# nighting0le01/On_Device_Image_Captioning

Measured on AMD Instinct MI355X. Metric: captions/sec end-to-end (Swin-L 384, beam=3) at 1/2/4/8 MI355X, higher is better.
Workload: dtype bf16; 1 GPU; End_ExpansionNet_v2 end-to-end, Swin-L/384 backbone, batch 16 per GPU, beam 3, beam_max_seq_len 20 (BASELINE.json configs[2]); workload_key=e2e16, batch_per_gpu=16, beam=3, beam_max_seq_len=20, decoder_steps=19, weights=synthetic xavier (Philox, seed 0), backbone_precision=bf16, encoder_precision=bf16, decoder_precision=fp32, hip_graphs=True, parallelism=image-shard x1, caption_len_check=20, encode_lanes=1, decode_lanes=2, decode_cus=0, decode_group_batches=1

## Files before the change

### include/odic_hip.h

```cpp
#ifndef ODIC_HIP_H
#define ODIC_HIP_H

#include <stddef.h>
#include <stdint.h>

#ifdef __cplusplus
extern "C" {
#endif

#define ODIC_F32 0
#define ODIC_BF16 1
#define ODIC_FP8 2
#define ODIC_F16 3
#define ODIC_H2 4

#define ODIC_ACT_NONE 0
#define ODIC_ACT_GELU 1
#define ODIC_ACT_RELU 2
#define ODIC_ACT_SIGMOID 3

#define ODIC_EINVAL (-1)
#define ODIC_ENULL (-2)
#define ODIC_EUNSUPPORTED (-3)

#define ODIC_ABI_VERSION 23
int odic_abi_version(void);

const char* odic_build_info(void);

typedef struct odic_gemm_args {
  const void* A; const void* W; const float* bias; const float* residual; void* out;
  int32_t M, N, K;
  int64_t lda, ldw, ldr, ldc;
  int32_t batch;
  int64_t strideA, strideW, strideBias, strideR, strideC;
  float alpha;
  int32_t act;
  int32_t bias_axis;
  int32_t in_dtype;
  int32_t out_dtype;
  int32_t tile_cfg;
  const float* ln_colsum; float ln_eps;
  int32_t* workspace;
  const float* col_scale; float out_scale;
  void* out16; int64_t ld16; float* stats_out;
  const float* ln_stats;
  const float* a_ln; int64_t ld_aln;
} odic_gemm_args;
int odic_gemm(const odic_gemm_args* args, void* stream);

int odic_layernorm(const float* x, int64_t ldx, const float* gamma, const float* beta, void* out,
                   int32_t M, int32_t C, float eps, int32_t out_dtype, void* stream);

int odic_copy(const void* src, void* dst, int64_t nbytes, void* stream);

int odic_cast_f32_to_bf16(const float* x, int64_t ldx, void* out, int64_t ldo, int32_t M, int32_t C,
                          void* stream);
int odic_cast_f32_to_h2(const float* x, int64_t ldx, void* out, int64_t ldo, int32_t M, int32_t C, void* stream);
// ... 76 lines not shown
} odic_jpeg_scan;

typedef struct odic_jpeg_prog_batch {
  const void* headers;
  const void* scans;
  const void* tables;
  const uint8_t* data;
  uint8_t* out;
  int32_t* status;
  int32_t n_images, n_scans, n_tables, n_levels, max_width, max_height, pad0, pad1;
  int64_t max_blocks, total_scan_bytes, total_intervals, total_blocks, total_plane_bytes;
  int32_t level_first[ODIC_JPEG_MAX_SCANS + 1];
  int32_t level_intervals[ODIC_JPEG_MAX_SCANS];
  int32_t pad2;
} odic_jpeg_prog_batch;

size_t odic_jpeg_progressive_workspace_bytes(const odic_jpeg_prog_batch* batch);

size_t odic_jpeg_progressive_coef_offset(const odic_jpeg_prog_batch* batch);

int odic_jpeg_decode_progressive(const odic_jpeg_prog_batch* batch, void* workspace, size_t ws_bytes, void* stream);

int odic_jpeg_decode_progressive_scaled(const odic_jpeg_prog_batch* batch, const int32_t* scale_log2, void* workspace,
                                        size_t ws_bytes, void* stream);

int odic_window_attention(const void* qkv, const float* bias_table, const float* bias_shifted_prescaled,
                          void* out, int32_t B, int32_t res, int32_t C, int32_t heads, int32_t ws,
                          int32_t shift, float scale, int32_t dtype, void* stream);

int odic_swin_qkv_attention(const float* x, int64_t ldx, const void* w_qkv_folded, const float* b_qkv_folded,
                            const float* bias_shifted_prescaled, void* out, int32_t B, int32_t res, int32_t C,
                            int32_t heads, int32_t ws, int32_t shift, float scale, float ln_eps, void* stream);

int odic_swin_mlp(const float* x, int64_t ldx, const void* w1_folded, const float* b1_folded, const void* w2,
                  const float* b2, float alpha2, float* out, int64_t ldo, int32_t M, int32_t C, float ln_eps,
                  void* stream);

int odic_stcexp_normalize(const float* z, const int32_t* enc_len, const int32_t* group_meta,
                          int32_t ngroups, void* pos_fw, void* neg_fw, int64_t ld_fw, void* pos_bw,
                          void* neg_bw, int64_t ld_bw, float* colsum_ws, int32_t B, int32_t nq,
                          int32_t S, float eps, float scale_fw, float scale_bw, int32_t out_dtype, void* stream);

int odic_selector_mix(const float* x, int64_t ldx, const float* sel_pre, int64_t lds,
                      const float* a, int64_t lda, const float* b, int64_t ldb, float* out,
                      int64_t ldo, int32_t M, int32_t d, void* stream);


int odic_dec_embed(const int64_t* tokens, const float* embed, const float* pos_table,
                   const int32_t* pos, float* y, int64_t ldy, int32_t N, int32_t d, int32_t pos_rows,
                   float scale, void* stream);

int odic_dynexp_step(const float* lin, int64_t ldlin, const float* qexp, const float* bexp,
                     float* cond_c, float* key_c, float* va_c, float* vb_c, float* wfa_c,
                     float* wfb_c, float* qk_c, const int32_t* anc, const int32_t* row_valid,
                     const int32_t* pos, const float* y_in, int64_t ldy_in, float* y, int64_t ldy,
                     int32_t N, int32_t T, int32_t d, int32_t E, float eps, void* stream);


int odic_dec_embed_seq(const int64_t* tokens, const float* embed, const float* pos_table, const int32_t* dec_len,
                       int32_t* row_valid, float* y, int64_t ldy, int32_t N, int32_t T, int32_t d, int32_t vocab,
                       int32_t pos_rows, float scale, void* stream);

int odic_dynexp_seq(const float* lin, int64_t ldlin, const float* qexp, const float* bexp, const int32_t* dec_len,
                    const float* y_in, int64_t ldy_in, float* y, int64_t ldy, int32_t N, int32_t T, int32_t d,
                    int32_t E, float eps, void* stream);

// ... 54 lines not shown
```

### on_device_image_captioning_amd/_hip.py

```python
from __future__ import annotations

import ctypes as C
import os

_HERE = os.path.dirname(os.path.abspath(__file__))
LIB_PATH = os.path.join(_HERE, "libodic_hip.so")

F32, BF16, FP8, F16, H2 = 0, 1, 2, 3, 4
ACT_NONE, ACT_GELU, ACT_RELU, ACT_SIGMOID = 0, 1, 2, 3
ABI_VERSION = 23

_ERR = {-1: "ODIC_EINVAL (bad shape / alignment / enum)", -2: "ODIC_ENULL (required pointer is NULL)",
        -3: "ODIC_EUNSUPPORTED"}


class GemmArgs(C.Structure):
    _fields_ = [("A", C.c_void_p), ("W", C.c_void_p), ("bias", C.c_void_p), ("residual", C.c_void_p),
                ("out", C.c_void_p),
                ("M", C.c_int32), ("N", C.c_int32), ("K", C.c_int32),
                ("lda", C.c_int64), ("ldw", C.c_int64), ("ldr", C.c_int64), ("ldc", C.c_int64),
                ("batch", C.c_int32),
                ("strideA", C.c_int64), ("strideW", C.c_int64), ("strideBias", C.c_int64),
                ("strideR", C.c_int64), ("strideC", C.c_int64),
                ("alpha", C.c_float), ("act", C.c_int32), ("bias_axis", C.c_int32),
                ("in_dtype", C.c_int32), ("out_dtype", C.c_int32), ("tile_cfg", C.c_int32),
                ("ln_colsum", C.c_void_p), ("ln_eps", C.c_float), ("workspace", C.c_void_p),
                ("col_scale", C.c_void_p), ("out_scale", C.c_float),
                ("out16", C.c_void_p), ("ld16", C.c_int64), ("stats_out", C.c_void_p), ("ln_stats", C.c_void_p),
                ("a_ln", C.c_void_p), ("ld_aln", C.c_int64)]


class BeamState(C.Structure):
    _fields_ = [(n, C.c_void_p) for n in
                ("tokens", "logprobs", "anc", "cumul", "n_elem", "has_eos", "row_valid", "next_tok",
                 "pos", "done", "ctr")]


class EmbedArgs(C.Structure):
    _fields_ = [("embed", C.c_void_p), ("pos_table", C.c_void_p), ("y", C.c_void_p), ("ldy", C.c_int64),
                ("d", C.c_int32), ("scale", C.c_float), ("pos_rows", C.c_int32)]


class JpegBatch(C.Structure):
# ... 7 lines not shown


JPEG_MAX_SCANS = 64


class JpegProgBatch(C.Structure):
    _fields_ = [("headers", C.c_void_p), ("scans", C.c_void_p), ("tables", C.c_void_p), ("data", C.c_void_p),
                ("out", C.c_void_p), ("status", C.c_void_p),
                ("n_images", C.c_int32), ("n_scans", C.c_int32), ("n_tables", C.c_int32), ("n_levels", C.c_int32),
                ("max_width", C.c_int32), ("max_height", C.c_int32), ("pad0", C.c_int32), ("pad1", C.c_int32),
                ("max_blocks", C.c_int64), ("total_scan_bytes", C.c_int64), ("total_intervals", C.c_int64),
                ("total_blocks", C.c_int64), ("total_plane_bytes", C.c_int64),
                ("level_first", C.c_int32 * (JPEG_MAX_SCANS + 1)), ("level_intervals", C.c_int32 * JPEG_MAX_SCANS),
                ("pad2", C.c_int32)]


_P, _I32, _I64, _F = C.c_void_p, C.c_int32, C.c_int64, C.c_float

_SIGNATURES = {
    "odic_abi_version": (C.c_int, []),
    "odic_build_info": (C.c_char_p, []),
    "odic_gemm": (C.c_int, [C.POINTER(GemmArgs), _P]),
    "odic_layernorm": (C.c_int, [_P, _I64, _P, _P, _P, _I32, _I32, _F, _I32, _P]),
    "odic_cast_f32_to_bf16": (C.c_int, [_P, _I64, _P, _I64, _I32, _I32, _P]),
    "odic_cast_f32_to_h2": (C.c_int, [_P, _I64, _P, _I64, _I32, _I32, _P]),
    "odic_patch_merge_layernorm": (C.c_int, [_P, _P, _P, _P, _I32, _I32, _I32, _F, _I32, _P]),
    "odic_patch_embed": (C.c_int, [_P] * 6 + [_I32] * 6 + [_F, _P]),
    "odic_resize_bilinear_normalize": (C.c_int, [_P, _I32, _I32, _I64, _P, _P, _I32, _P, _P, _I32, _P, _P, _I32,
                                                 C.POINTER(C.c_float), C.POINTER(C.c_float), _P]),
    "odic_resize_boxes_normalize": (C.c_int, [_P, _I32, _P, _P, _P, _P, C.c_size_t, _P, _I32, _I32,
                                              C.POINTER(C.c_float), C.POINTER(C.c_float), _P]),
    "odic_window_attention": (C.c_int, [_P, _P, _P, _P] + [_I32] * 6 + [_F, _I32, _P]),
    "odic_swin_qkv_attention": (C.c_int, [_P, _I64, _P, _P, _P, _P] + [_I32] * 6 + [_F, _F, _P]),
    "odic_swin_mlp": (C.c_int, [_P, _I64, _P, _P, _P, _P, _F, _P, _I64, _I32, _I32, _F, _P]),
    "odic_stcexp_normalize": (C.c_int, [_P, _P, _P, _I32, _P, _P, _I64, _P, _P, _I64, _P, _I32, _I32, _I32, _F, _F, _F, _I32,
                                        _P]),
    "odic_selector_mix": (C.c_int, [_P, _I64, _P, _I64, _P, _I64, _P, _I64, _P, _I64, _I32, _I32, _P]),
    "odic_copy": (C.c_int, [_P, _P, _I64, _P]),
    "odic_dec_embed": (C.c_int, [_P, _P, _P, _P, _P, _I64, _I32, _I32, _I32, _F, _P]),
    "odic_dec_embed_seq": (C.c_int, [_P, _P, _P, _P, _P, _P, _I64] + [_I32] * 5 + [_F, _P]),
    "odic_dynexp_seq": (C.c_int, [_P, _I64, _P, _P, _P, _P, _I64, _P, _I64] + [_I32] * 4 + [_F, _P]),
    "odic_token_stats": (C.c_int, [_P, _I64, _P, _P, _P, _P, _P, _P, _I32, _I32, _P]),
    "odic_dynexp_step": (C.c_int, [_P, _I64, _P, _P] + [_P] * 7 + [_P, _P, _P, _P, _I64, _P, _I64] + [_I32] * 4 + [_F, _P]),
    "odic_cross_attn_step": (C.c_int, [_P, _I64, _P, _I64, _I32, _I32, _P, _P, _P, _I64] + [_I32] * 5 + [_P]),
    "odic_cross_attn_probs": (C.c_int, [_P, _I64, _P, _I64, _I32, _P, _P, _P, _I64] + [_I32] * 7 + [_F, _P]),
    "odic_logsoftmax_topk": (C.c_int, [_P, _I64, _P, _I64, _P, _P, _I32, _I32, _I32, _P]),
    "odic_logsoftmax_sample": (C.c_int, [_P, _I64, _P, _I64, _P, _P, _I32, _I32, _I32, C.c_uint64, _P, _P]),
    "odic_ensemble_logprobs": (C.c_int, [C.POINTER(C.c_void_p), _I32, _I64, _P, _I64, _I32, _I32, _P]),
    "odic_topk_rows": (C.c_int, [_P, _I64, _P, _P, _I32, _I32, _I32, _P]),
    "odic_beam_step": (C.c_int, [_P, _P, C.POINTER(BeamState), C.POINTER(EmbedArgs), _I32, _I32, _I32, _I64, _P]),
    "odic_beam_finalize": (C.c_int, [C.POINTER(BeamState), _P, _P, _I32, _I32, _P]),
    "odic_beam_finalize_best": (C.c_int, [C.POINTER(BeamState), _P, _P, _P, _P, _I32, _I32, _I32, _I32, _P]),
    "odic_beam_reset": (C.c_int, [C.POINTER(BeamState), C.POINTER(EmbedArgs), _I32, _I32, _I32, _I64, _P]),
    "odic_jpeg_workspace_bytes": (C.c_size_t, [C.POINTER(JpegBatch)]),
    "odic_jpeg_decode": (C.c_int, [C.POINTER(JpegBatch), _P, C.c_size_t, _P]),
    "odic_jpeg_progressive_workspace_bytes": (C.c_size_t, [C.POINTER(JpegProgBatch)]),
    "odic_jpeg_progressive_coef_offset": (C.c_size_t, [C.POINTER(JpegProgBatch)]),
    "odic_jpeg_decode_progressive": (C.c_int, [C.POINTER(JpegProgBatch), _P, C.c_size_t, _P]),
    "odic_jpeg_decode_scaled": (C.c_int, [C.POINTER(JpegBatch), _P, _P, C.c_size_t, _P]),
    "odic_jpeg_decode_progressive_scaled": (C.c_int, [C.POINTER(JpegProgBatch), _P, _P, C.c_size_t, _P]),
}

EXPORTED_SYMBOLS = tuple(_SIGNATURES)

_lib = None

# ... 28 lines not shown
```

### on_device_image_captioning_amd/csrc/window_attention.hip

```cpp
#include "gemm_tile.h"

namespace {

constexpr int HD = 32;
constexpr int MAXN = 144;

struct WinGeom {
  int B, res, C, heads, ws, shift, nwin_side;
  float scale;
};
struct WinParams {
  const void* qkv; const float* table; const float* bias_shifted; void* out;
  WinGeom g;
};

struct Window { int b, wy, wx; };
__device__ __forceinline__ Window window_of(const WinGeom& g, int win) {
  const int wpi = g.nwin_side * g.nwin_side;
  const int b = win / wpi, wrem = win - b * wpi;
  const int wy = wrem / g.nwin_side, wx = wrem - wy * g.nwin_side;
  return {b, wy, wx};
}
__device__ __forceinline__ bool on_shift_seam(const WinGeom& g, const Window& w) {
  return g.shift > 0 && (w.wy == g.nwin_side - 1 || w.wx == g.nwin_side - 1);
// ... 603 lines not shown
    bf16x4_t pk[9];
#pragma unroll
    for (int kt = 0; kt < 9; ++kt) {
#pragma unroll
      for (int hh = 0; hh < 2; ++hh) {
        const f32x2_t a = f32x2_t{sc[kt][2 * hh], sc[kt][2 * hh + 1]} * s2 + c2;
        const f32x2_t e = {__builtin_amdgcn_exp2f(a[0]), __builtin_amdgcn_exp2f(a[1])};
        lsum += e;
        pk[kt][2 * hh] = (short)f32_to_bf16(e[0]);
        pk[kt][2 * hh + 1] = (short)f32_to_bf16(e[1]);
      }
    }
    float l = lsum[0] + lsum[1];
    l += __shfl_xor(l, 16, 64);
    l += __shfl_xor(l, 32, 64);
    const float inv_l = __builtin_amdgcn_rcpf(l);
    f32x4_t oacc[2] = {f32x4_t{0.f, 0.f, 0.f, 0.f}, f32x4_t{0.f, 0.f, 0.f, 0.f}};
#pragma unroll
    for (int s5 = 0; s5 < 5; ++s5) {
      const bf16x4_t lo4 = pk[2 * s5];
      const bf16x4_t hi4 = s5 < 4 ? pk[2 * s5 + (s5 < 4)] : bf16x4_t{0, 0, 0, 0};
      const bf16x8_t pf = bf16x8_t{lo4[0], lo4[1], lo4[2], lo4[3], hi4[0], hi4[1], hi4[2], hi4[3]};
#pragma unroll
      for (int nt = 0; nt < 2; ++nt) {
        const v4s_t lo = __builtin_amdgcn_ds_read_tr16_b64_v4i16(
            (__attribute__((address_space(3))) v4s_t*)(vbase + (32 * s5) * HD * 2 + nt * 32));
        const v4s_t hi = __builtin_amdgcn_ds_read_tr16_b64_v4i16(
            (__attribute__((address_space(3))) v4s_t*)(vbase + (32 * s5 + 16) * HD * 2 + nt * 32));
        const bf16x8_t vf = bf16x8_t{lo[0], lo[1], lo[2], lo[3], hi[0], hi[1], hi[2], hi[3]};
        oacc[nt] = __builtin_amdgcn_mfma_f32_16x16x32_bf16(vf, pf, oacc[nt], 0, 0, 0);
      }
    }
    store_o16<false>(p.out + (long)orow * C + h * HD + fq * 4, oacc, inv_l);
  }
}


__global__ __launch_bounds__(192, 3) void window_attention_h2_kernel(WinParams p) {
  __shared__ __attribute__((aligned(16))) char Kx[MAXN * 128];
  __shared__ __attribute__((aligned(16))) bf16_raw Vh[MAXN + 16][HD];
  __shared__ __attribute__((aligned(16))) bf16_raw Vl[MAXN + 16][HD];
  __shared__ __attribute__((aligned(16))) float Bs[4 * BS_COPY];
  __shared__ int rows[MAXN];
  __shared__ __attribute__((aligned(4))) unsigned char rids[MAXN];

  ODIC_ENCODE_PRIO();
  const int xcd = blockIdx.x & 7, idx = blockIdx.x >> 3;
  const int head = idx % p.g.heads;
  const int win = (idx / p.g.heads) * 8 + xcd;
  if (win >= p.g.B * (p.g.nwin_side * p.g.nwin_side)) return;
  const Window w = window_of(p.g, win);
  const int tid = threadIdx.x, lane = tid & 63, wave = tid >> 6;
  const char* qkv = (const char*)p.qkv;
  const long ldb = 12L * p.g.C;
  const long kbyte = 4L * p.g.C, vbyte = 8L * p.g.C;
  const bool masked = on_shift_seam(p.g, w);

  {
    const float* bsrc = p.bias_shifted + (long)head * 4 * BS_COPY + lane * 4;
#pragma unroll
    for (int i = 0; i < 3; ++i) {
      const int blk = wave * 3 + i;
      __builtin_amdgcn_global_load_lds((gptr_t)(bsrc + blk * 256), (lptr_t)((char*)&Bs[0] + blk * 1024), 16, 0, 0);
    }
  }
  stage_rows(p.g, w, tid, rows, rids);
// ... 146 lines not shown
    if (packed) hipLaunchKernelGGL(window_attention_bf16_v3_kernel<false>, xgrid, block, 0, s, p);
    else hipLaunchKernelGGL(window_attention_bf16_kernel, grid, block, 0, s, p);
  } else if (dtype == ODIC_F16) {
    if (ws != 12 || !packed) return ODIC_EUNSUPPORTED;
    hipLaunchKernelGGL(window_attention_bf16_v3_kernel<true>, xgrid, block, 0, s, p);
  } else if (dtype == ODIC_H2) {
    if (ws != 12 || !packed || ((uintptr_t)qkv & 31) || ((uintptr_t)out & 31))
      return ODIC_EUNSUPPORTED;
    hipLaunchKernelGGL(window_attention_h2_kernel, xgrid, block, 0, s, p);
  } else {
    return ODIC_EINVAL;
  }
  return odic_launch_status();
}

extern "C" int odic_swin_qkv_attention(const float* x, int64_t ldx, const void* w_qkv_folded, const float* b_qkv_folded,
                                       const float* bias_shifted_prescaled, void* out, int32_t B, int32_t res, int32_t C,
                                       int32_t heads, int32_t ws, int32_t shift, float scale, float ln_eps, void* stream) {
  if (!x || !w_qkv_folded || !b_qkv_folded || !bias_shifted_prescaled || !out) return ODIC_ENULL;
  if (B <= 0 || ws != 12 || res % ws || heads * HD != C || shift < 0 || shift >= ws || ldx < C) return ODIC_EINVAL;
  if (C != 192) return ODIC_EUNSUPPORTED;
  if (((uintptr_t)x & 15) || (ldx & 3) || ((uintptr_t)w_qkv_folded & 15) || ((uintptr_t)out & 7) ||
      ((uintptr_t)bias_shifted_prescaled & 15) || ((uintptr_t)b_qkv_folded & 3) || (long)B * res * res >= 2147483647L)
    return ODIC_EINVAL;
  const FusedParams p = {x, ldx, (const bf16_raw*)w_qkv_folded, b_qkv_folded, bias_shifted_prescaled, (bf16_raw*)out,
                         {B, res, C, heads, ws, shift, res / ws, scale}, ln_eps};
  constexpr int SHMEM = 2 * 3 * 96 * 128 + MAXN * HD * 2 + (MAXN + 16) * HD * 2 + 2 * 4 * BS_COPY * 4 + 3 * 192 * 4 + MAXN * 4 + MAXN;
  auto k = swin_qkv_attention_kernel<3>;
  static bool done = false;
  if (!done) { (void)hipFuncSetAttribute((const void*)k, hipFuncAttributeMaxDynamicSharedMemorySize, SHMEM); done = true; }
  hipLaunchKernelGGL(k, dim3(B * p.g.nwin_side * p.g.nwin_side), dim3(576), SHMEM, (hipStream_t)stream, p);
  return odic_launch_status();
}
```

### on_device_image_captioning_amd/engine.py

```python
from __future__ import annotations

import ctypes as C
import math
import os
from typing import Dict, List, Optional, Sequence, Tuple

import torch

from . import _hip, ops
from .weights import Geometry

SD = Dict[str, torch.Tensor]
_CDT = {"fp32": torch.float32, "bf16": torch.bfloat16, "fp8": torch.bfloat16, "x3": ops.H2_DTYPE}


def pack_operand(t: torch.Tensor, cdt) -> Tuple[torch.Tensor, float]:
    if cdt == ops.H2_DTYPE:
        sc = ops.pow2_scale_for_h2(t)
        return ops.h2_from_f32(t * sc), 1.0 / sc
    return t.to(cdt).contiguous(), 1.0


def _dev(t: torch.Tensor, device, dtype=None) -> torch.Tensor:
    t = t.detach()
# ... 16 lines not shown
        self.pe_w = _dev(sd[f"{P}.patch_embed.proj.weight"].reshape(g.swin_embed_dim, -1), device, torch.float32)
        self.pe_b = f32(f"{P}.patch_embed.proj.bias")
        self.pe_g, self.pe_beta = f32(f"{P}.patch_embed.norm.weight"), f32(f"{P}.patch_embed.norm.bias")
        self.stages = []
        for s, depth in enumerate(g.swin_depths):
            blocks = []
            for b in range(depth):
                p = f"{P}.layers.{s}.blocks.{b}"
                (qkv_w, qkv_a), (proj_w, proj_a) = cw(p + ".attn.qkv.weight"), cw(p + ".attn.proj.weight")
                (fc1_w, fc1_a), (fc2_w, fc2_a) = cw(p + ".mlp.fc1.weight"), cw(p + ".mlp.fc2.weight")
                blocks.append(dict(
                    n1w=f32(p + ".norm1.weight"), n1b=f32(p + ".norm1.bias"),
                    qkv_w=qkv_w, qkv_a=qkv_a, qkv_b=f32(p + ".attn.qkv.bias"),
                    table=f32(p + ".attn.relative_position_bias_table"),
                    dense=(ops.shifted_bias_prescaled(f32(p + ".attn.relative_position_bias_table"), g.stage_window(s),
                                                      (g.stage_dim(s) // g.swin_num_heads[s]) ** -0.5)
                           if fast_attn and g.stage_window(s) == 12 else None),
                    proj_w=proj_w, proj_a=proj_a, proj_b=f32(p + ".attn.proj.bias"),
                    n2w=f32(p + ".norm2.weight"), n2b=f32(p + ".norm2.bias"),
                    fc1_w=fc1_w, fc1_a=fc1_a, fc1_b=f32(p + ".mlp.fc1.bias"),
                    fc2_w=fc2_w, fc2_a=fc2_a, fc2_b=f32(p + ".mlp.fc2.bias"),
                    shift=g.stage_shift(s, b)))
            down = None
            if s < len(g.swin_depths) - 1:
                p = f"{P}.layers.{s}.downsample"
                red_w, red_a = cw(p + ".reduction.weight")
                down = dict(nw=f32(p + ".norm.weight"), nb=f32(p + ".norm.bias"), red_w=red_w, red_a=red_a)
            self.stages.append((blocks, down))
        self.fn_w, self.fn_b = f32(f"{P}.norm.weight"), f32(f"{P}.norm.bias")
        self.stage_chunks = [int(v) for v in os.environ.get("ODIC_SWIN_CHUNKS", "1").split(",")]
        lr = os.environ.get("ODIC_FUSE_BACKBONE_LN_READ", "1")
        self.ln_read = (precision == "bf16" and lr != "0") or (precision == "x3" and lr == "x3")
        self.fuse_qkv_attn = precision == "bf16" and os.environ.get("ODIC_FUSE_QKV_ATTENTION", "1") == "1"
        self.fuse_mlp = precision == "bf16" and os.environ.get("ODIC_FUSE_MLP", "1") == "1"
        if self.ln_read:
            for s, (blocks, _) in enumerate(self.stages):
                if g.stage_dim(s) != 192:
                    continue
                for b, w in enumerate(blocks):
                    p = f"{P}.layers.{s}.blocks.{b}"
                    if precision == "bf16":
                        w["qkv_lnr"] = ops.fold_layernorm_bf16(f32(p + ".attn.qkv.weight"), w["qkv_b"], w["n1w"], w["n1b"])[:2] + (1.0,)
                        w["fc1_lnr"] = ops.fold_layernorm_bf16(f32(p + ".mlp.fc1.weight"), w["fc1_b"], w["n2w"], w["n2b"])[:2] + (1.0,)
                    else:
                        for name, wk, bk, nw, nb in (("qkv_lnr", ".attn.qkv.weight", "qkv_b", "n1w", "n1b"),
                                                     ("fc1_lnr", ".mlp.fc1.weight", "fc1_b", "n2w", "n2b")):
                            Wg, b2, _ = ops.fold_layernorm(f32(p + wk), w[bk], w[nw], w[nb])
                            op, alpha = pack_operand(Wg, self.cdt)
                            w[name] = (op, b2, alpha)
        self.fp8_ready = False
        if fp8:
            self._pack_fp8(sd, calibration_images)

    def _pack_fp8(self, sd: SD, calibration_images) -> None:
        from .weights import synth_images
        g, dv = self.g, self.device
        if any(g.stage_window(s) != 12 or g.stage_dim(s) % 64 for s in range(len(g.swin_depths))):
            raise RuntimeError("fp8 mode needs 12x12 windows and stage widths that are multiples of 64 (Swin-L: 192·2^s)")
        img = calibration_images if calibration_images is not None else synth_images(2, g, seed=7)
        amax = {}
        self.forward(img.to(dv, torch.float32), _amax=amax)
        P = "swin_transf"
        margin = 1.25
        self.fp8_range = {k: margin * v for k, v in amax.items()}
        for s, (blocks, _) in enumerate(self.stages):
            for b, w in enumerate(blocks):
# ... 44 lines not shown
            x_all, B_all = x, B
            B = B_all // n_ch
            for ci, bi, w in ((ci, bi, w) for ci in range(n_ch) for bi, w in enumerate(blocks)):
                x = x_all[ci * B * res * res:(ci + 1) * B * res * res]
                if fp8:
                    xn = ops.layernorm(x, w["n1w8"], w["n1b8"], out_dtype=ops.FP8_DTYPE)
                    qkv = ops.gemm(xn, w["qkv_w8"], w["qkv_b"], col_scale=w["qkv_cs"], out_dtype=torch.float16)
                    att = ops.window_attention(qkv, w["table"], B, res, C_, heads, ws, w["shift"],
                                               bias_shifted_prescaled=w["dense"])
                    ops.gemm(att, w["proj_w16"], w["proj_b"], residual=x, out=x)
                    xn = ops.layernorm(x, w["n2w8"], w["n2b8"], out_dtype=ops.FP8_DTYPE)
                    h = ops.gemm(xn, w["fc1_w8"], w["fc1_b"], act=ops.ACT_GELU, col_scale=w["fc1_cs"],
                                 out_scale=w["hid_inv"], out_dtype=ops.FP8_DTYPE)
                    ops.gemm(h, w["fc2_w8"], w["fc2_b"], residual=x, out=x, col_scale=w["fc2_cs"])
                elif "qkv_lnr" in w and _amax is None and ops.a_ln_supported(x.shape[0], 3 * C_, C_, cdt):
                    if self.fuse_qkv_attn and ws == 12 and w["dense"] is not None:
                        att = ops.swin_qkv_attention(x, w["qkv_lnr"][0], w["qkv_lnr"][1], w["dense"], B, res, C_, heads,
                                                     ws, w["shift"])
                    else:
                        qkv = ops.gemm(None, w["qkv_lnr"][0], w["qkv_lnr"][1], a_ln=x, out_dtype=cdt, alpha=w["qkv_lnr"][2])
                        att = ops.window_attention(qkv, w["table"], B, res, C_, heads, ws, w["shift"],
                                                   bias_shifted_prescaled=w["dense"])
                    ops.gemm(att, w["proj_w"], w["proj_b"], residual=x, out=x, alpha=w["proj_a"])
                    if self.fuse_mlp and ops.swin_mlp_supported(x.shape[0], C_, cdt):
                        ops.swin_mlp(x, w["fc1_lnr"][0], w["fc1_lnr"][1], w["fc2_w"], w["fc2_b"], w["fc2_a"], out=x)
                    else:
                        h = ops.gemm(None, w["fc1_lnr"][0], w["fc1_lnr"][1], a_ln=x, act=ops.ACT_GELU, out_dtype=cdt,
                                     alpha=w["fc1_lnr"][2])
                        ops.gemm(h, w["fc2_w"], w["fc2_b"], residual=x, out=x, alpha=w["fc2_a"])
                else:
                    xn = ops.layernorm(x, w["n1w"], w["n1b"], out_dtype=cdt)
                    if _amax is not None:
                        _amax[(s, bi, "ln1")] = float(xn.float().abs().max())
                    qkv = ops.gemm(xn, w["qkv_w"], w["qkv_b"], alpha=w["qkv_a"])
                    att = ops.window_attention(qkv, w["table"], B, res, C_, heads, ws, w["shift"],
                                               bias_shifted_prescaled=w["dense"])
                    ops.gemm(att, w["proj_w"], w["proj_b"], residual=x, out=x, alpha=w["proj_a"])
                    xn = ops.layernorm(x, w["n2w"], w["n2b"], out_dtype=cdt)
                    h = ops.gemm(xn, w["fc1_w"], w["fc1_b"], act=ops.ACT_GELU, alpha=w["fc1_a"])
                    if _amax is not None:
                        _amax[(s, bi, "ln2")] = float(xn.float().abs().max())
                        _amax[(s, bi, "hid")] = float(h.float().abs().max())
                    ops.gemm(h, w["fc2_w"], w["fc2_b"], residual=x, out=x, alpha=w["fc2_a"])
                if taps is not None:
                    taps[f"s{s}b{bi}"] = x.view(B, res * res, C_).clone()
            x, B = x_all, B_all
            if down is not None:
                xm = ops.patch_merge_layernorm(x, down["nw"], down["nb"], B, res, C_, out_dtype=cdt)
                x = ops.gemm(xm.view(-1, 4 * C_), down["red_w"], out_dtype=torch.float32, alpha=down["red_a"])
                if taps is not None:
                    taps[f"merge{s}"] = x.view(B, (res // 2) ** 2, 2 * C_).clone()
        res = g.stage_res(len(g.swin_depths) - 1)
        out = ops.layernorm(x, self.fn_w, self.fn_b, out_dtype=out_dtype)
        return out.view(B, res * res, -1)


class DecodeState:

    def __init__(self, eng: "CaptionerEngine", n_img: int, beams: int, T: int, kv: torch.Tensor,
                 enc_len: torch.Tensor, S: int):
        g, dv = eng.g, eng.device
        N = n_img * beams
        d, E, L = g.d_model, g.num_exp_dec, g.N_dec
        self.n_img, self.beams, self.N, self.T, self.S = n_img, beams, N, T, S
        self.kv, self.enc_len = kv, enc_len
        f = lambda *s: torch.zeros(*s, dtype=torch.float32, device=dv)
        i32 = lambda *s: torch.zeros(*s, dtype=torch.int32, device=dv)
        self.ycat = f(N, L * d)
        self.caches = [dict(cond=f(T, N, d), key=f(T, N, d), va=f(T, N, d), vb=f(T, N, d),
# ... 318 lines not shown
```

### on_device_image_captioning_amd/ops.py

```python
from __future__ import annotations

import ctypes as C
import os
from typing import Optional, Sequence

import torch

from . import _hip
from ._hip import ACT_GELU, ACT_NONE, ACT_RELU, ACT_SIGMOID, BF16, F16, F32, FP8, H2

FP8_DTYPE = torch.float8_e4m3fn
FP8_MAX = 448.0
H2_DTYPE = torch.int32
_DT = {torch.float32: F32, torch.bfloat16: BF16, torch.float16: F16, FP8_DTYPE: FP8, H2_DTYPE: H2}


def _stream() -> C.c_void_p:
    return C.c_void_p(torch.cuda.current_stream().cuda_stream)


_PROFILE: Optional[list] = None


class profile:
# ... 345 lines not shown
    return out


def shifted_bias_prescaled(bias_table: torch.Tensor, ws: int, scale: float) -> torch.Tensor:
    if ws != 12:
        raise RuntimeError("the packed bias layout is specialised for 12x12 windows")
    heads = bias_table.shape[1]
    t = (bias_table.double() / scale).float().view(23, 23, heads)
    R = torch.zeros(heads, 23 * 24 + 32, dtype=torch.float32, device=bias_table.device)
    R[:, :23 * 24].view(heads, 23, 24)[:, :, :23] = t.flip(1).permute(2, 0, 1)
    out = torch.zeros(heads, 4, 576, dtype=torch.float32, device=bias_table.device)
    for s_ in range(4):
        out[:, s_, :] = R[:, s_:s_ + 576]
    return out.contiguous()


def swin_qkv_attention(x: torch.Tensor, w_folded: torch.Tensor, b_folded: torch.Tensor, bias_shifted_prescaled: torch.Tensor,
                       B: int, res: int, C_: int, heads: int, ws: int, shift: int, *, eps: float = 1e-5,
                       out: Optional[torch.Tensor] = None) -> torch.Tensor:
    _need_cuda(x, w_folded, b_folded, bias_shifted_prescaled, out)
    if x.dtype != torch.float32 or w_folded.dtype != torch.bfloat16 or not (x.is_contiguous() and w_folded.is_contiguous()):
        raise RuntimeError("swin_qkv_attention: contiguous fp32 rows and a contiguous bf16 folded weight")
    if out is None:
        out = torch.empty(B * res * res, C_, dtype=torch.bfloat16, device=x.device)
    nwh = B * (res // ws) ** 2 * heads
    with _timed("swin_qkv_attention", 2.0 * B * res * res * C_ * 3 * C_ + nwh * 2654208.0,
                B * res * res * C_ * (4 + 2) + 3 * C_ * C_ * 2, f"res{res}h{heads}"):
        _hip.check(_hip.load().odic_swin_qkv_attention(_p(x), C_, _p(w_folded), _p(b_folded), _p(bias_shifted_prescaled),
                                                      _p(out), B, res, C_, heads, ws, shift, (C_ // heads) ** -0.5, eps,
                                                      _stream()), "odic_swin_qkv_attention")
    return out


def swin_mlp_supported(M: int, C_: int, dtype=torch.bfloat16) -> bool:
    return dtype == torch.bfloat16 and C_ == 192 and M > 0 and M % 128 == 0


def swin_mlp(x: torch.Tensor, w1_folded: torch.Tensor, b1_folded: torch.Tensor, w2: torch.Tensor, b2: torch.Tensor,
             alpha2: float = 1.0, out: Optional[torch.Tensor] = None, ln_eps: float = 1e-5) -> torch.Tensor:
    _need_cuda(x, w1_folded, b1_folded, w2, b2, out)
    if x.dtype != torch.float32 or w1_folded.dtype != torch.bfloat16 or w2.dtype != torch.bfloat16 or \
            not (x.is_contiguous() and w1_folded.is_contiguous() and w2.is_contiguous()):
        raise RuntimeError("swin_mlp: contiguous fp32 rows and contiguous bf16 weights")
    C_ = x.shape[-1]
    M = x.numel() // C_
    if tuple(w1_folded.shape) != (4 * C_, C_) or tuple(w2.shape) != (C_, 4 * C_) or b1_folded.numel() != 4 * C_ or \
            b2.numel() != C_ or b1_folded.dtype != torch.float32 or b2.dtype != torch.float32:
        raise RuntimeError("swin_mlp: fc1 is [4C, C] with an fp32 bias [4C], fc2 [C, 4C] with an fp32 bias [C]")
    if out is None:
        out = torch.empty_like(x)
    elif out.dtype != torch.float32 or out.shape != x.shape or not out.is_contiguous():
        raise RuntimeError("swin_mlp: out is a contiguous fp32 tensor of x's shape")
    with _timed("swin_mlp", 2.0 * M * C_ * 4 * C_ * 2, 2.0 * M * C_ * 4 + 2 * 4 * C_ * C_ * 2, f"{M}x{C_}"):
        _hip.check(_hip.load().odic_swin_mlp(_p(x), C_, _p(w1_folded), _p(b1_folded), _p(w2), _p(b2), float(alpha2), _p(out),
                                             C_, M, C_, float(ln_eps), _stream()), "odic_swin_mlp")
    return out


def window_attention(qkv: torch.Tensor, bias_table: torch.Tensor, B: int, res: int, C_: int, heads: int, ws: int,
                     shift: int, *, scale: Optional[float] = None, out: Optional[torch.Tensor] = None,
                     bias_shifted_prescaled: Optional[torch.Tensor] = None) -> torch.Tensor:
    _need_cuda(qkv, bias_table, out, bias_shifted_prescaled)
    if scale is None:
        scale = (C_ // heads) ** -0.5
    if out is None:
        out = torch.empty((B * res * res, C_), dtype=qkv.dtype, device=qkv.device)
# ... 183 lines not shown
```

Baseline: 1965 captions/s.

## Add tiled fused QKV GEMM plus window attention kernel for wide Swin stages

Adds a kernel that computes the QKV projection for a 144-row window tile across three heads with MFMA. It then runs windowed softmax attention on the result in LDS, so the qkv tensor is never written to or read back from global memory. It is enabled by default for stages with C >= 768 (Swin-L stages 3/4), where it replaces the separate qkv GEMM and window_attention launches. The cost is high LDS use with one block per CU, 576 threads per block, and a weight tile that is reloaded for every window.

```diff
diff --git a/include/odic_hip.h b/include/odic_hip.h
--- a/include/odic_hip.h
+++ b/include/odic_hip.h
@@ -23,7 +23,7 @@
 #define ODIC_ENULL (-2)
 #define ODIC_EUNSUPPORTED (-3)
 
-#define ODIC_ABI_VERSION 23
+#define ODIC_ABI_VERSION 24
 int odic_abi_version(void);
 
 const char* odic_build_info(void);
@@ -166,6 +166,10 @@
                             const float* bias_shifted_prescaled, void* out, int32_t B, int32_t res, int32_t C,
                             int32_t heads, int32_t ws, int32_t shift, float scale, float ln_eps, void* stream);
 
+int odic_swin_qkv_attention_tiled(const void* xn, const void* w_qkv, const float* b_qkv,
+                                  const float* bias_shifted_prescaled, void* out, int32_t B, int32_t res, int32_t C,
+                                  int32_t heads, int32_t ws, int32_t shift, float scale, void* stream);
+
 int odic_swin_mlp(const float* x, int64_t ldx, const void* w1_folded, const float* b1_folded, const void* w2,
                   const float* b2, float alpha2, float* out, int64_t ldo, int32_t M, int32_t C, float ln_eps,
                   void* stream);
diff --git a/on_device_image_captioning_amd/_hip.py b/on_device_image_captioning_amd/_hip.py
--- a/on_device_image_captioning_amd/_hip.py
+++ b/on_device_image_captioning_amd/_hip.py
@@ -8,7 +8,7 @@
 
 F32, BF16, FP8, F16, H2 = 0, 1, 2, 3, 4
 ACT_NONE, ACT_GELU, ACT_RELU, ACT_SIGMOID = 0, 1, 2, 3
-ABI_VERSION = 23
+ABI_VERSION = 24
 
 _ERR = {-1: "ODIC_EINVAL (bad shape / alignment / enum)", -2: "ODIC_ENULL (required pointer is NULL)",
         -3: "ODIC_EUNSUPPORTED"}
@@ -82,6 +82,7 @@
                                               C.POINTER(C.c_float), C.POINTER(C.c_float), _P]),
     "odic_window_attention": (C.c_int, [_P, _P, _P, _P] + [_I32] * 6 + [_F, _I32, _P]),
     "odic_swin_qkv_attention": (C.c_int, [_P, _I64, _P, _P, _P, _P] + [_I32] * 6 + [_F, _F, _P]),
+    "odic_swin_qkv_attention_tiled": (C.c_int, [_P] * 5 + [_I32] * 6 + [_F, _P]),
     "odic_swin_mlp": (C.c_int, [_P, _I64, _P, _P, _P, _P, _F, _P, _I64, _I32, _I32, _F, _P]),
     "odic_stcexp_normalize": (C.c_int, [_P, _P, _P, _I32, _P, _P, _I64, _P, _P, _I64, _P, _I32, _I32, _I32, _F, _F, _F, _I32,
                                         _P]),
diff --git a/on_device_image_captioning_amd/csrc/window_attention.hip b/on_device_image_captioning_amd/csrc/window_attention.hip
--- a/on_device_image_captioning_amd/csrc/window_attention.hip
+++ b/on_device_image_captioning_amd/csrc/window_attention.hip
@@ -659,6 +659,234 @@
       }
     }
     store_o16<false>(p.out + (long)orow * C + h * HD + fq * 4, oacc, inv_l);
+  }
+}
+
+
+struct TiledParams {
+  const bf16_raw* A; const bf16_raw* W; const float* bqkv; const float* bias_shifted; bf16_raw* out;
+  WinGeom g;
+  TileGrid grid;
+};
+
+constexpr int QT_ROWB = 128, QT_A_BYTES = 144 * QT_ROWB, QT_W_BYTES = 288 * QT_ROWB, QT_STAGE = QT_A_BYTES + QT_W_BYTES;
+constexpr int QT_KIMG = MAXN * HD * 2, QT_VIMG = (MAXN + 16) * HD * 2, QT_BIMG = 4 * BS_COPY * 4;
+constexpr int QT_SHMEM = 2 * QT_STAGE + 144 * 8;
+static_assert(3 * QT_BIMG + 3 * QT_KIMG <= QT_STAGE && 3 * QT_VIMG <= QT_STAGE, "the core's images reuse the two stages");
+static_assert(MAXN * 4 + MAXN <= 144 * 8, "rows[] and rids[] fit the tail");
+
+__global__ __launch_bounds__(576, 1) void swin_qkv_attention_tiled_kernel(TiledParams p) {
+  constexpr int NW = 9, NWN = 3, MI = 3, NI = 6, BK = 64;
+  constexpr int ROWB = QT_ROWB, A_BYTES = QT_A_BYTES, STAGE = QT_STAGE;
+  constexpr int A_INSTR = 2, W_INSTR = 4;
+  extern __shared__ __attribute__((aligned(16))) char lds[];
+  int* rows = (int*)(lds + 2 * STAGE);
+  unsigned char* rids = (unsigned char*)(rows + MAXN);
+
+  const int tid = threadIdx.x, lane = tid & 63;
+  const int wave = __builtin_amdgcn_readfirstlane(tid >> 6);
+  const int wm = wave / NWN, wn = wave % NWN;
+  ODIC_ENCODE_PRIO();
+
+  int tm, tn;
+  {
+    const int xcd = blockIdx.x & 7, idx = blockIdx.x >> 3;
+    const int xm = xcd / p.grid.pn, xn = xcd - xm * p.grid.pn;
+    const int r0 = xm * p.grid.tiles_m / p.grid.pm, r1 = (xm + 1) * p.grid.tiles_m / p.grid.pm;
+    const int c0 = xn * p.grid.tiles_n / p.grid.pn, c1 = (xn + 1) * p.grid.tiles_n / p.grid.pn;
+    const int w = c1 - c0;
+    if (idx >= (r1 - r0) * w) return;
+    const int lr = idx / w;
+    tm = r0 + lr; tn = c0 + (idx - lr * w);
+  }
+  const int C = p.g.C;
+  const Window w = window_of(p.g, tm);
+  const bool masked = on_shift_seam(p.g, w);
+  const int head = 3 * tn + wn;
+  stage_rows(p.g, w, tid, rows, rids);
+
+  const int srow = lane >> 3;
+  const int schunk = swz<ROWB>(lane & 7, srow);
+  const bf16_raw* a_src[A_INSTR];
+  const bf16_raw* w_src[W_INSTR];
+#pragma unroll
+  for (int i = 0; i < A_INSTR; ++i) {
+    long r; int rid;
+    slot_to_token(p.g, w, (i * NW + wave) * 8 + srow, r, rid);
+    a_src[i] = p.A + r * C + schunk * 8;
+  }
+#pragma unroll
+  for (int i = 0; i < W_INSTR; ++i) {
+    const int row = (i * NW + wave) * 8 + srow;
+    const int wc = row / 96, rem = row - wc * 96;
+    w_src[i] = p.W + (long)((rem >> 5) * C + (3 * tn + wc) * HD + wperm(rem & 31)) * C + schunk * 8;
+  }
+
+  auto stage = [&](int buf, int kt) {
+    char* la = lds + buf * STAGE;
+    char* lw = la + A_BYTES;
+#pragma unroll
+    for (int i = 0; i < A_INSTR; ++i)
+      __builtin_amdgcn_global_load_lds((gptr_t)(a_src[i] + (long)kt * BK), (lptr_t)(la + (i * NW + wave) * 1024), 16, 0, 0);
+#pragma unroll
+    for (int i = 0; i < W_INSTR; ++i)
+      __builtin_amdgcn_global_load_lds((gptr_t)(w_src[i] + (long)kt * BK), (lptr_t)(lw + (i * NW + wave) * 1024), 16, 0, 0);
+  };
+
+  f32x4_t acc[MI][NI];
+#pragma unroll
+  for (int i = 0; i < MI; ++i)
+#pragma unroll
+    for (int j = 0; j < NI; ++j) acc[i][j] = f32x4_t{0.f, 0.f, 0.f, 0.f};
+
+  const int nk = C / BK;
+  const int frow = lane & 15, fq = lane >> 4;
+  char* Bp = lds + (nk & 1) * STAGE;
+  char* Kp = Bp + 3 * QT_BIMG;
+  char* Vp = lds + ((nk & 1) ^ 1) * STAGE;
+
+  stage(0, 0);
+  for (int kt = 0; kt < nk; ++kt) {
+    asm volatile("s_waitcnt vmcnt(0)" ::: "memory");
+    __builtin_amdgcn_s_barrier();
+    if (kt + 1 < nk) {
+      stage((kt + 1) & 1, kt + 1);
+    } else {
+      const float* bsrc = p.bias_shifted + (long)(3 * tn) * 4 * BS_COPY + lane * 4;
+#pragma unroll
+      for (int i = 0; i < 3; ++i)
+        __builtin_amdgcn_global_load_lds((gptr_t)(bsrc + (i * NW + wave) * 256), (lptr_t)(Bp + (i * NW + wave) * 1024), 16, 0, 0);
+    }
+
+    const int cur = kt & 1;
+    const char* la = lds + cur * STAGE + (wm * MI * 16 + frow) * ROWB;
+    const char* lw = lds + cur * STAGE + A_BYTES + (wn * NI * 16 + frow) * ROWB;
+#pragma unroll
+    for (int kk = 0; kk < BK / 32; ++kk) {
+      bf16x8_t af[MI], wf[NI];
+      const int chunk = swz<ROWB>(kk * 4 + fq, frow) << 4;
+#pragma unroll
+      for (int mi = 0; mi < MI; ++mi) af[mi] = *(const bf16x8_t*)(la + mi * 16 * ROWB + chunk);
+#pragma unroll
+      for (int ni = 0; ni < NI; ++ni) wf[ni] = *(const bf16x8_t*)(lw + ni * 16 * ROWB + chunk);
+#pragma unroll
+      for (int mi = 0; mi < MI; ++mi)
+#pragma unroll
+        for (int ni = 0; ni < NI; ++ni)
+          acc[mi][ni] = __builtin_amdgcn_mfma_f32_16x16x32_bf16(wf[ni], af[mi], acc[mi][ni], 0, 0, 0);
+    }
+  }
+
+  bf16x8_t qf[MI], kf8[MI], vf8[MI];
+  {
+    f32x4_t bc[3][2];
+#pragma unroll
+    for (int u = 0; u < 3; ++u) {
+      const f32x4_t* bp = (const f32x4_t*)(p.bqkv + u * C + head * HD + fq * 8);
+      bc[u][0] = bp[0]; bc[u][1] = bp[1];
+    }
+#pragma unroll
+    for (int mi = 0; mi < MI; ++mi) {
+      bf16x8_t o[3];
+#pragma unroll
+      for (int u = 0; u < 3; ++u) {
+        const f32x4_t v0 = acc[mi][2 * u] * 1.0f + bc[u][0], v1 = acc[mi][2 * u + 1] * 1.0f + bc[u][1];
+#pragma unroll
+        for (int e = 0; e < 4; ++e) { o[u][e] = (short)f32_to_bf16(v0[e]); o[u][4 + e] = (short)f32_to_bf16(v1[e]); }
+      }
+      qf[mi] = o[0]; kf8[mi] = o[1]; vf8[mi] = o[2];
+    }
+  }
+  asm volatile("s_waitcnt lgkmcnt(0)" ::: "memory");
+  __builtin_amdgcn_s_barrier();
+  {
+    char* kimg = Kp + wn * QT_KIMG;
+    char* vimg = Vp + wn * QT_VIMG;
+#pragma unroll
+    for (int mi = 0; mi < MI; ++mi) {
+      const int slot = (wm * MI + mi) * 16 + frow;
+      *(bf16x8_t*)(kimg + slot * HD * 2 + ((fq ^ ((frow >> 2) & 3)) << 4)) = kf8[mi];
+      *(bf16x8_t*)(vimg + slot * HD * 2 + (fq << 4)) = vf8[mi];
+    }
+    if (tid < 3 * 128) ((unsigned long long*)(Vp + (tid >> 7) * QT_VIMG + MAXN * HD * 2))[tid & 127] = 0ull;
+  }
+  asm volatile("s_waitcnt vmcnt(0) lgkmcnt(0)" ::: "memory");
+  __builtin_amdgcn_s_barrier();
+
+  const float scale2 = p.g.scale * 1.4426950408889634f;
+  const float mask_acc = 100.0f / p.g.scale;
+  const int voff = ((4 * fq + (frow >> 2)) * HD + 4 * (frow & 3)) * 2;
+  int koffs[9];
+#pragma unroll
+  for (int kt = 0; kt < 9; ++kt) {
+    const int key0 = kt * 16 + fq * 4;
+    const int jy = key0 / 12, jx0 = key0 - jy * 12;
+    koffs[kt] = (jx0 - jy * 24) * 4;
+  }
+  auto bias_base = [&](int qn) -> int {
+    const int iy = qn / 12, ix = qn - iy * 12;
+    const int s = (11 - ix) & 3;
+    return (s * BS_COPY + (iy + 11) * 24 + 11 - ix - s) * 4;
+  };
+#pragma unroll
+  for (int qt = 0; qt < 3; ++qt) {
+    const int qn = (wm * 3 + qt) * 16 + frow;
+    const int orow = rows[qn];
+    int koff = (frow * HD + ((fq ^ ((frow >> 2) & 3)) * 8)) * 2, vo = voff, bb = bias_base(qn);
+    opaque_offsets(koff, vo, bb);
+    const char* kbase = Kp + wn * QT_KIMG + koff;
+    const char* vbase = Vp + wn * QT_VIMG + vo;
+    const char* bbase = Bp + wn * QT_BIMG + bb;
+    f32x4_t sc[9];
+    load_bias36(bbase, koffs, sc);
+    scores16<false>(kbase, qf[qt], sc);
+    if (masked) {
+      const unsigned my = rids[qn];
+#pragma unroll
+      for (int kt = 0; kt < 9; ++kt) {
+        const unsigned kr = *(const unsigned*)&rids[kt * 16 + fq * 4];
+#pragma unroll
+        for (int j = 0; j < 4; ++j)
+          if (((kr >> (8 * j)) & 0xff) != my) sc[kt][j] -= mask_acc;
+      }
+    }
+    const float m = row_max36(sc);
+    const f32x2_t s2 = {scale2, scale2};
+    const f32x2_t c2 = {-m * scale2, -m * scale2};
+    f32x2_t lsum = {0.f, 0.f};
+    bf16x4_t pk[9];
+#pragma unroll
+    for (int kt = 0; kt < 9; ++kt) {
+#pragma unroll
+      for (int h = 0; h < 2; ++h) {
+        const f32x2_t a = f32x2_t{sc[kt][2 * h], sc[kt][2 * h + 1]} * s2 + c2;
+        const f32x2_t e = {__builtin_amdgcn_exp2f(a[0]), __builtin_amdgcn_exp2f(a[1])};
+        lsum += e;
+        pk[kt][2 * h] = (short)f32_to_bf16(e[0]);
+        pk[kt][2 * h + 1] = (short)f32_to_bf16(e[1]);
+      }
+    }
+    float l = lsum[0] + lsum[1];
+    l += __shfl_xor(l, 16, 64);
+    l += __shfl_xor(l, 32, 64);
+    const float inv_l = __builtin_amdgcn_rcpf(l);
+    f32x4_t oacc[2] = {f32x4_t{0.f, 0.f, 0.f, 0.f}, f32x4_t{0.f, 0.f, 0.f, 0.f}};
+#pragma unroll
+    for (int s5 = 0; s5 < 5; ++s5) {
+      const bf16x4_t lo4 = pk[2 * s5];
+      const bf16x4_t hi4 = s5 < 4 ? pk[2 * s5 + (s5 < 4)] : bf16x4_t{0, 0, 0, 0};
+      const bf16x8_t pf = bf16x8_t{lo4[0], lo4[1], lo4[2], lo4[3], hi4[0], hi4[1], hi4[2], hi4[3]};
+#pragma unroll
+      for (int nt = 0; nt < 2; ++nt) {
+        const v4s_t lo = __builtin_amdgcn_ds_read_tr16_b64_v4i16(
+            (__attribute__((address_space(3))) v4s_t*)(vbase + (32 * s5) * HD * 2 + nt * 32));
+        const v4s_t hi = __builtin_amdgcn_ds_read_tr16_b64_v4i16(
+            (__attribute__((address_space(3))) v4s_t*)(vbase + (32 * s5 + 16) * HD * 2 + nt * 32));
+        const bf16x8_t vf = bf16x8_t{lo[0], lo[1], lo[2], lo[3], hi[0], hi[1], hi[2], hi[3]};
+        oacc[nt] = __builtin_amdgcn_mfma_f32_16x16x32_bf16(vf, pf, oacc[nt], 0, 0, 0);
+      }
+    }
+    store_o16<false>(p.out + (long)orow * C + head * HD + fq * 4, oacc, inv_l);
   }
 }
 
@@ -871,3 +1099,21 @@
   hipLaunchKernelGGL(k, dim3(B * p.g.nwin_side * p.g.nwin_side), dim3(576), SHMEM, (hipStream_t)stream, p);
   return odic_launch_status();
 }
+
+extern "C" int odic_swin_qkv_attention_tiled(const void* xn, const void* w_qkv, const float* b_qkv,
+                                             const float* bias_shifted_prescaled, void* out, int32_t B, int32_t res,
+                                             int32_t C, int32_t heads, int32_t ws, int32_t shift, float scale, void* stream) {
+  if (!xn || !w_qkv || !b_qkv || !bias_shifted_prescaled || !out) return ODIC_ENULL;
+  if (B <= 0 || res <= 0 || ws <= 0 || heads <= 0 || res % ws || shift < 0 || shift >= ws) return ODIC_EINVAL;
+  if (ws != 12 || heads * HD != C || heads % 3 || C % 64) return ODIC_EUNSUPPORTED;
+  if (((uintptr_t)xn & 15) || ((uintptr_t)w_qkv & 15) || ((uintptr_t)out & 7) || ((uintptr_t)bias_shifted_prescaled & 15) ||
+      ((uintptr_t)b_qkv & 15) || (long)B * res * res >= 2147483647L)
+    return ODIC_EINVAL;
+  TiledParams p = {(const bf16_raw*)xn, (const bf16_raw*)w_qkv, b_qkv, bias_shifted_prescaled, (bf16_raw*)out,
+                   {B, res, C, heads, ws, shift, res / ws, scale}, {}};
+  const long M = (long)B * res * res;
+  const int max_rect = tile_grid(p.grid, (int)M, 3 * C, 144, 288, (double)M * C * 2.0, 3.0 * C * C * 2.0, 32);
+  tile_allow_lds<QT_SHMEM, swin_qkv_attention_tiled_kernel>();
+  hipLaunchKernelGGL(swin_qkv_attention_tiled_kernel, dim3(8 * max_rect), dim3(576), QT_SHMEM, (hipStream_t)stream, p);
+  return odic_launch_status();
+}
diff --git a/on_device_image_captioning_amd/engine.py b/on_device_image_captioning_amd/engine.py
--- a/on_device_image_captioning_amd/engine.py
+++ b/on_device_image_captioning_amd/engine.py
@@ -72,6 +72,8 @@
         lr = os.environ.get("ODIC_FUSE_BACKBONE_LN_READ", "1")
         self.ln_read = (precision == "bf16" and lr != "0") or (precision == "x3" and lr == "x3")
         self.fuse_qkv_attn = precision == "bf16" and os.environ.get("ODIC_FUSE_QKV_ATTENTION", "1") == "1"
+        self.fuse_qkv_attn_tiled = precision == "bf16" and os.environ.get("ODIC_FUSE_QKV_ATTENTION_TILED", "1") == "1"
+        self.fuse_qkv_attn_tiled_min_c = int(os.environ.get("ODIC_FUSE_QKV_ATTENTION_TILED_MIN_C", "768"))
         self.fuse_mlp = precision == "bf16" and os.environ.get("ODIC_FUSE_MLP", "1") == "1"
         if self.ln_read:
             for s, (blocks, _) in enumerate(self.stages):
@@ -182,9 +184,15 @@
                     xn = ops.layernorm(x, w["n1w"], w["n1b"], out_dtype=cdt)
                     if _amax is not None:
                         _amax[(s, bi, "ln1")] = float(xn.float().abs().max())
-                    qkv = ops.gemm(xn, w["qkv_w"], w["qkv_b"], alpha=w["qkv_a"])
-                    att = ops.window_attention(qkv, w["table"], B, res, C_, heads, ws, w["shift"],
-                                               bias_shifted_prescaled=w["dense"])
+                    if (self.fuse_qkv_attn_tiled and _amax is None and w["dense"] is not None and w["qkv_a"] == 1.0
+                            and C_ >= self.fuse_qkv_attn_tiled_min_c
+                            and ops.swin_qkv_attention_tiled_supported(x.shape[0], C_, heads, ws, res, cdt)):
+                        att = ops.swin_qkv_attention_tiled(xn, w["qkv_w"], w["qkv_b"], w["dense"], B, res, C_, heads, ws,
+                                                           w["shift"])
+                    else:
+                        qkv = ops.gemm(xn, w["qkv_w"], w["qkv_b"], alpha=w["qkv_a"])
+                        att = ops.window_attention(qkv, w["table"], B, res, C_, heads, ws, w["shift"],
+                                                   bias_shifted_prescaled=w["dense"])
                     ops.gemm(att, w["proj_w"], w["proj_b"], residual=x, out=x, alpha=w["proj_a"])
                     xn = ops.layernorm(x, w["n2w"], w["n2b"], out_dtype=cdt)
                     h = ops.gemm(xn, w["fc1_w"], w["fc1_b"], act=ops.ACT_GELU, alpha=w["fc1_a"])
diff --git a/on_device_image_captioning_amd/ops.py b/on_device_image_captioning_amd/ops.py
--- a/on_device_image_captioning_amd/ops.py
+++ b/on_device_image_captioning_amd/ops.py
@@ -401,6 +401,29 @@
     return out
 
 
+def swin_qkv_attention_tiled_supported(M: int, C_: int, heads: int, ws: int, res: int, dtype=torch.bfloat16) -> bool:
+    return (dtype == torch.bfloat16 and ws == 12 and heads > 0 and heads * 32 == C_ and heads % 3 == 0 and C_ % 64 == 0
+            and res > 0 and res % ws == 0 and M > 0 and M % (res * res) == 0)
+
+
+def swin_qkv_attention_tiled(xn: torch.Tensor, w_qkv: torch.Tensor, b_qkv: torch.Tensor, bias_shifted_prescaled: torch.Tensor,
+                             B: int, res: int, C_: int, heads: int, ws: int, shift: int, *,
+                             out: Optional[torch.Tensor] = None) -> torch.Tensor:
+    _need_cuda(xn, w_qkv, b_qkv, bias_shifted_prescaled, out)
+    if (xn.dtype != torch.bfloat16 or w_qkv.dtype != torch.bfloat16 or not (xn.is_contiguous() and w_qkv.is_contiguous())
+            or xn.numel() != B * res * res * C_ or w_qkv.numel() != 3 * C_ * C_):
+        raise RuntimeError("swin_qkv_attention_tiled: contiguous bf16 rows [B·res², C] and a contiguous bf16 weight [3C, C]")
+    if out is None:
+        out = torch.empty(B * res * res, C_, dtype=torch.bfloat16, device=xn.device)
+    nwh = B * (res // ws) ** 2 * heads if ws > 0 else 0
+    with _timed("swin_qkv_attention", 2.0 * B * res * res * C_ * 3 * C_ + nwh * 2654208.0,
+                B * res * res * C_ * (2 + 2) + 3 * C_ * C_ * 2 + 3 * C_ * 4 + heads * 9216, f"res{res}h{heads}"):
+        _hip.check(_hip.load().odic_swin_qkv_attention_tiled(_p(xn), _p(w_qkv), _p(b_qkv), _p(bias_shifted_prescaled), _p(out),
+                                                            B, res, C_, heads, ws, shift, (C_ // heads) ** -0.5 if heads > 0 else 0.0,
+                                                            _stream()), "odic_swin_qkv_attention_tiled")
+    return out
+
+
 def swin_mlp_supported(M: int, C_: int, dtype=torch.bfloat16) -> bool:
     return dtype == torch.bfloat16 and C_ == 192 and M > 0 and M % 128 == 0
 
```

Measured after the change: 2064 captions/s (median of 6 runs). 1.05x the previous value.
